# tarepan/ForwardTacotron

Measured on AMD Instinct MI355X. Metric: mel-frames/sec at batch=64 LJSpeech shapes (ForwardTacotron.generate, B*T_mel per s), higher is better.
Workload: dtype fp32; 1 GPU; c3: ForwardTacotron generate, batch=64 per GPU, phoneme lengths U{50..200}; global_batch=64, T_phonemes=200, T_mel=1368, parallelism=dp1

## Files before the change

### forwardtacotron_amd/csrc/rnn.hip

```cpp
#include "common.h"

#ifdef FTMI_RNN_STAMPS
__device__ unsigned long long ftmi_rnn_stamps[2048 * 8];
#define STAMP(i)                                                                      \
  do {                                                                                \
    if (threadIdx.x == 0) {                                                           \
      __builtin_amdgcn_sched_barrier(0);                                              \
      unsigned long long now__;                                                       \
      asm volatile("s_waitcnt vmcnt(0) lgkmcnt(0)\n\ts_memtime %0\n\ts_waitcnt lgkmcnt(0)" \
                   : "=s"(now__)::"memory");                                         \
      __builtin_amdgcn_sched_barrier(0);                                              \
      st_acc[i] += now__ - st_last;                                                   \
      st_last = now__;                                                                \
    }                                                                                 \
  } while (0)
#else
#define STAMP(i) \
  do {           \
  } while (0)
#endif
#ifdef FTMI_DIAG
#define RNN_DIAG(p) ((p).diag)
#else
#define RNN_DIAG(p) ((void)(p), 0u)
#endif

namespace {

typedef __bf16 bf16x8 __attribute__((ext_vector_type(8)));
typedef _Float16 f16x8 __attribute__((ext_vector_type(8)));

constexpr float H3_SCALE = 2048.f;
constexpr float H3_UNSCALE = 1.f / 2048.f;

constexpr int NB = 16;
constexpr int RED_STRIDE = NB + 1;
constexpr unsigned SPIN_LIMIT_DEFAULT = 1u << 22;
unsigned g_spin_limit = SPIN_LIMIT_DEFAULT;
constexpr unsigned STATUS_TIMEOUT = 4u;
constexpr int CNT_PAD = 32;
constexpr int WS_ERR = 0;
constexpr int WS_CENSUS = 1 * CNT_PAD;
constexpr int WS_ARRIVE = 9 * CNT_PAD;
constexpr int WS_FLAGS = 10 * CNT_PAD;
constexpr int FLAGS_PER_GROUP = 64;
constexpr int WS_GROUPS_OF(int ngroups) { return WS_FLAGS + ngroups * FLAGS_PER_GROUP; }

struct RnnParams {
  const float *xp;
  int64_t xp_stride;
  int T_src;
  const int32_t *index;
  const float *xp_zero;
  const float *w_hh;
  const float *b_hh;
  float *y;
  int64_t y_stride;
  const int32_t *lengths;
  float pad_value;
  float *hx;
  int B, T;
  int ngroups_total;
  int chunk0;
  int ngroups;
  int xcd_local;
  unsigned *ws;
  unsigned *status;
  unsigned spin_limit;
  int psleep;
  int diag;
};

constexpr int WS_CHUNK = 8;
static int64_t ws_chunks(int64_t B) { return (B + WS_CHUNK - 1) / WS_CHUNK; }
static int64_t ctl_bytes(int64_t nchunks) {
  return (WS_GROUPS_OF((int)(2 * nchunks)) + 2 * nchunks * CNT_PAD) * (int64_t)sizeof(unsigned);
}

static bool hx_fits(const RnnParams &p, int H, int64_t slab_words) {
  return 2 * (int64_t)p.ngroups_total * slab_words <= 2 * (2 * ws_chunks(p.B)) * NB * (int64_t)H;
}

__device__ __forceinline__ float fast_sigmoid(float x) {
  return __builtin_amdgcn_rcpf(1.0f + __expf(-x));
}
__device__ __forceinline__ float fast_tanh(float x) { return 2.0f * fast_sigmoid(2.0f * x) - 1.0f; }

__device__ __forceinline__ void split3x8(const float (&v)[8], bf16x8 &h1, bf16x8 &h2, bf16x8 &h3) {
  typedef float f32x8 __attribute__((ext_vector_type(8)));
  f32x8 x;
#pragma unroll
  for (int i = 0; i < 8; ++i) x[i] = v[i];
  h1 = __builtin_convertvector(x, bf16x8);
  const f32x8 r1 = x - __builtin_convertvector(h1, f32x8);
  h2 = __builtin_convertvector(r1, bf16x8);
  const f32x8 r2 = r1 - __builtin_convertvector(h2, f32x8);
  h3 = __builtin_convertvector(r2, bf16x8);
}

__device__ __forceinline__ void split2h8(const float (&v)[8], f16x8 &h, f16x8 &t) {
  typedef float f32x8 __attribute__((ext_vector_type(8)));
  f32x8 x;
#pragma unroll
  for (int i = 0; i < 8; ++i) x[i] = v[i];
  h = __builtin_convertvector(x, f16x8);
  t = __builtin_convertvector((x - __builtin_convertvector(h, f32x8)) * H3_SCALE, f16x8);
}

__device__ __forceinline__ unsigned h_tag(int t) { return (((unsigned)t >> 1) & 1u) ^ 1u; }

__device__ __forceinline__ unsigned xcc_id() {
  unsigned x;
  asm volatile("s_getreg_b32 %0, hwreg(HW_REG_XCC_ID)" : "=s"(x));
  return x & 7u;
}

__device__ __forceinline__ bool poll_ge(unsigned *w, unsigned target, unsigned limit) {
  unsigned spins = 0;
  while (__hip_atomic_load(w, __ATOMIC_RELAXED, __HIP_MEMORY_SCOPE_AGENT) < target) {
    __builtin_amdgcn_s_sleep(1);
    if (++spins > limit) return false;
  }
  return true;
}

__device__ __forceinline__ void report_timeout(const RnnParams &p) {
  __hip_atomic_store(p.ws + WS_ERR, 1u, __ATOMIC_RELAXED, __HIP_MEMORY_SCOPE_AGENT);
  if (p.status) atomicOr(p.status, STATUS_TIMEOUT);
}

template <int CELL, int H, int U, int WK, int MODE, bool CST = false, int NBL = NB>
__global__ __launch_bounds__(H / U == 1 ? 256 : 320, 1) void rnn_bidir_kernel(
    const RnnParams p) {
  constexpr bool X6 = MODE != 0;
  constexpr bool H3 = MODE == 2;
  constexpr int G = CELL ? 4 : 3;
  constexpr int R = G * U;
  constexpr int RB = (R + 15) / 16;
  constexpr int WR = 4 / WK;
  constexpr int RBW = RB / WR;
  constexpr int KW = H / WK;
  constexpr int NL = KW / 16;
  constexpr int KS = KW / 32;
  constexpr int KB = KW / 4;
  constexpr int BPG = H / U;
  constexpr bool LOCAL = BPG == 1;
  constexpr int CELLS = U * NB;
  constexpr bool HALFCELL = CELLS < 256;
  constexpr int CPT = HALFCELL ? 1 : CELLS / 256;
  static_assert((R % 16 == 0 || U == 8) && (U % 16 == 0 || U == 8) && H % U == 0 &&
                    RB % WR == 0 && (CELLS % 256 == 0 || CELLS == 128), "shape");
  static_assert(X6 ? (KW % 32 == 0) : (KB % 4 == 0), "K split");
  static_assert(!CST || (H3 && !LOCAL && CPT == 1 && (U == 16 || U == 8)), "compute-wave h stores");
  static_assert(U != 8 || (CST && CELL == 0 && NBL == NB), "U = 8: the spread GRU's CST form");
  static_assert(NBL == NB || (NBL == 8 && !LOCAL), "live sequences per group");
  constexpr int RR = RB * 16;
  constexpr float GSC = H3 ? H3_UNSCALE : 1.f;

  __shared__ __attribute__((aligned(16))) float red[WK * RR * RED_STRIDE];
  __shared__ __attribute__((aligned(16))) float hloc[LOCAL ? 2 * 16 * H : 4];
  __shared__ __attribute__((aligned(16))) float hstage[LOCAL ? 4 : CELLS];
  __shared__ __attribute__((aligned(16))) float ystage[LOCAL ? 4 : CELLS];
  __shared__ int s_abort, s_group, s_bi, s_mode;

  const int tid = threadIdx.x, lane = tid & 63, wave = tid >> 6;
  const int wk = wave % WK, wr = wave / WK;
  const int ls = lane >> 4, lc = lane & 15;

  if (tid == 0) {
    int mode = 0, group = blockIdx.x % p.ngroups, bi = blockIdx.x / p.ngroups, abort = 0;
    if (!LOCAL && p.xcd_local) {
      const unsigned x = xcc_id();
      const unsigned slot = __hip_atomic_fetch_add(p.ws + WS_CENSUS + x * CNT_PAD, 1u,
                                                   __ATOMIC_RELAXED, __HIP_MEMORY_SCOPE_AGENT);
      __hip_atomic_fetch_add(p.ws + WS_ARRIVE, 1u, __ATOMIC_RELAXED, __HIP_MEMORY_SCOPE_AGENT);
      if (!poll_ge(p.ws + WS_ARRIVE, gridDim.x, p.spin_limit)) {
        abort = 1;
        report_timeout(p);
      } else if (p.ngroups % 8 == 0 || (int)gridDim.x == 8 * BPG) {
        const int gpx = p.ngroups % 8 == 0 ? p.ngroups / 8 : 1;
        const unsigned per = (unsigned)gpx * BPG;
        bool balanced = true;
        for (int i = 0; i < 8; ++i)
          balanced &= __hip_atomic_load(p.ws + WS_CENSUS + i * CNT_PAD, __ATOMIC_RELAXED,
                                        __HIP_MEMORY_SCOPE_AGENT) == per;
        if (balanced) {
          mode = 1;
          group = (int)(x * gpx + slot / BPG);
          bi = (int)(slot % BPG);
        }
      }
    }
    s_mode = mode;
    s_group = group;
    s_bi = bi;
    s_abort = abort;
  }
  __syncthreads();
  if (s_abort) return;
  if (s_group >= p.ngroups || s_bi >= BPG) return;
  const int group = s_group, bi = s_bi;
  const bool xcd_mode = s_mode == 1;
  const int dir = group & 1;
  const int chunk = p.chunk0 + (group >> 1);
  const int gglob = p.chunk0 * 2 + group;
  const int u0 = bi * U;
  unsigned *cnt = p.ws + WS_GROUPS_OF(p.ngroups_total) + gglob * CNT_PAD;
  unsigned *flags = p.ws + WS_FLAGS + gglob * FLAGS_PER_GROUP;
  static_assert(BPG <= FLAGS_PER_GROUP, "flags");

  if constexpr (!LOCAL) {
    if (wave == 4) {
      constexpr int F4 = CELLS / 4;
      constexpr int FPL = F4 < 64 ? 1 : F4 / 64;
      static_assert(F4 % 64 == 0 || F4 == 32, "comm wave tiling");
      const auto rs = __builtin_amdgcn_make_buffer_rsrc(p.hx, (short)0, 0x7FFFFFF0, 0x00020000);
      const int hxp = p.ngroups_total * 16 * H * 4;
      unsigned hofs[FPL];
      int yb[FPL], k0s[FPL];
      bool ok[FPL];
#pragma unroll
      for (int i = 0; i < FPL; ++i) {
        const int f = lane + 64 * i;
        {
          const int bl = f / (U / 4);
          yb[i] = chunk * NBL + bl;
          k0s[i] = u0 + (f % (U / 4)) * 4;
          ok[i] = f < F4 && bl < NBL && yb[i] < p.B;
        }
        if constexpr (H3) {
          const int bl = f / (U / 4), rem = f % (U / 4), plane = rem & 1;
          const int k0 = u0 + (rem >> 1) * 8;
          const int kwv = k0 / KW, r = k0 % KW, q = r % 32;
          const int ln = (q >> 3) * 16 + bl;
          hofs[i] = (unsigned)((gglob * 16 * H * 2 +
                                ((kwv * NL + (r / 32) * 2 + plane) * 64 + ln) * 8) * 2);
        } else {
          const int bl = f / (U / 4);
          const int k0 = u0 + (f % (U / 4)) * 4;
          const int kwv = k0 / KW, r = k0 % KW;
          int ln, idx4;
          if constexpr (X6) {
            const int q = r % 32;
            ln = (q >> 3) * 16 + bl;
            idx4 = (r / 32) * 2 + ((q & 7) >> 2);
          } else {
            ln = (r / KB) * 16 + bl;
            idx4 = (r % KB) >> 2;
          }
          hofs[i] = (unsigned)((gglob * 16 * H + ((kwv * NL + idx4) * 64 + ln) * 4) * 4);
        }
      }
      __syncthreads();
      for (int t = 0; t < p.T; ++t) {
        const int tt = dir ? (p.T - 1 - t) : t;
        __syncthreads();
        if (s_abort) break;
        __syncthreads();
        const int soff = (t & 1) * hxp;
        typedef unsigned u32x4 __attribute__((ext_vector_type(4)));
#pragma unroll
        for (int i = 0; i < (CST ? 0 : FPL); ++i) {
          const u32x4 v = *(const u32x4 *)&hstage[(lane + 64 * i) * 4];
          if (NBL != NB && (lane + 64 * i) / (U / 4) >= NBL) continue;
          if (xcd_mode)
            __builtin_amdgcn_raw_buffer_store_b128(v, rs, hofs[i], soff, 0);
          else
            __builtin_amdgcn_raw_buffer_store_b128(v, rs, hofs[i], soff, 16);
        }
#pragma unroll
        for (int i = 0; i < FPL; ++i) {
          const f32x4 v = *(const f32x4 *)&ystage[((lane + 64 * i) % F4) * 4];
          if (ok[i]) *(f32x4 *)(p.y + ((size_t)yb[i] * p.T + tt) * p.y_stride + dir * H + k0s[i]) = v;
        }
      }
      return;
    }
  }

  const float *wdir = p.w_hh + (size_t)dir * (G * H) * H;
  bf16x8 wa[(X6 && !H3) ? RBW : 1][(X6 && !H3) ? KS : 1][3];
  f16x8 wh[H3 ? RBW : 1][H3 ? KS : 1][2];
  float wf[X6 ? 1 : RBW][X6 ? 1 : KB];
  bool wbad = false;
#pragma unroll
  for (int i = 0; i < RBW; ++i) {
    const int lrow0 = (wr * RBW + i) * 16 + lc;
    const bool rlive = lrow0 < R;
    const int lrow = rlive ? lrow0 : 0;
    const int grow = (lrow / U) * H + u0 + (lrow % U);
    const float *src = wdir + (size_t)grow * H + wk * KW;
    if constexpr (X6) {
#pragma unroll
      for (int ks = 0; ks < KS; ++ks) {
        float v[8];
        const f32x4 a = *(const f32x4 *)(src + ks * 32 + 8 * ls);
        const f32x4 b = *(const f32x4 *)(src + ks * 32 + 8 * ls + 4);
        v[0] = a.x; v[1] = a.y; v[2] = a.z; v[3] = a.w;
        v[4] = b.x; v[5] = b.y; v[6] = b.z; v[7] = b.w;
        if (!rlive)
#pragma unroll
          for (int e = 0; e < 8; ++e) v[e] = 0.f;
        if constexpr (H3) {
          split2h8(v, wh[i][ks][0], wh[i][ks][1]);
#pragma unroll
          for (int e = 0; e < 8; ++e) wbad |= !(__builtin_fabsf(v[e]) <= 65504.f);
        } else {
          split3x8(v, wa[i][ks][0], wa[i][ks][1], wa[i][ks][2]);
        }
      }
    } else {
#pragma unroll
      for (int kb = 0; kb < KB; kb += 4) {
        const f32x4 v = *(const f32x4 *)(src + ls * KB + kb);
        wf[i][kb] = v.x;
        wf[i][kb + 1] = v.y;
        wf[i][kb + 2] = v.z;
        wf[i][kb + 3] = v.w;
      }
    }
  }

  if (wbad && p.status) atomicOr(p.status, 2u);

  int cu[CPT], cb[CPT], cbl[CPT], len[CPT], hxo[CPT];
  bool cvalid[CPT];
  float hstate[CPT], cstate[CPT], bhh[CPT][G];
#pragma unroll
  for (int j = 0; j < CPT; ++j) {
    const int c = tid + 256 * j;
    cu[j] = c % U;
    const int bl = c / U;
    cbl[j] = bl;
    cb[j] = chunk * NBL + bl;
    cvalid[j] = bl < NBL && cb[j] < p.B;
    hstate[j] = 0.f;
    cstate[j] = 0.f;
    len[j] = (p.lengths && cvalid[j]) ? p.lengths[cb[j]] : p.T;
#pragma unroll
    for (int g = 0; g < G; ++g) {
      bhh[j][g] = (CELL == 0) ? p.b_hh[dir * G * H + g * H + u0 + cu[j]] : 0.f;
    }
    const int k = u0 + cu[j];
    const int kwv = k / KW, r = k % KW;
    int ln, idx4, e;
    if constexpr (X6) {
      const int q = r % 32;
      ln = (q >> 3) * 16 + bl;
      idx4 = (r / 32) * 2 + ((q & 7) >> 2);
      e = q & 3;
    } else {
      ln = (r / KB) * 16 + bl;
      idx4 = (r % KB) >> 2;
      e = r & 3;
    }
    hxo[j] = ((kwv * NL + idx4) * 64 + ln) * 4 + e;
  }

  const int slab = 16 * H;
  const auto rsrc = __builtin_amdgcn_make_buffer_rsrc(p.hx, (short)0, 0x7FFFFFF0, 0x00020000);
  const unsigned hoff = (unsigned)((gglob * slab + wk * NL * 256 + lane * 4) * 4);
  const int hx_par = p.ngroups_total * slab * 4;
  unsigned cst_off = 0;
  if constexpr (CST) {
    const int f = 16 * wave + (lane & 15);
    const int bl = f / (U / 4), rem = f % (U / 4), plane = rem & 1;
    const int k0 = u0 + (rem >> 1) * 8;
    const int kwv = k0 / KW, r = k0 % KW, q = r % 32;
    const int ln = (q >> 3) * 16 + bl;
    cst_off = (unsigned)((gglob * 16 * H * 2 + ((kwv * NL + (r / 32) * 2 + plane) * 64 + ln) * 8) * 2);
  }

  const int32_t *iptr[CPT];
  size_t brow[CPT];
#pragma unroll
  for (int j = 0; j < CPT; ++j) {
    const int b = cvalid[j] ? cb[j] : 0;
    iptr[j] = p.index ? p.index + (size_t)b * p.T : (const int32_t *)p.ws;
    brow[j] = (size_t)b * p.T_src;
  }
  const float *xcol = p.xp + dir * G * H + u0;
  const float *zcol = (p.index ? p.xp_zero : p.xp) + dir * G * H + u0;
  auto frame = [&](int t) { return dir ? (p.T - 1 - t) : t; };
  auto load_idx = [&](int t, int (&ir)[CPT]) {
    const int tt = frame(t < p.T ? t : p.T - 1);
#pragma unroll
    for (int j = 0; j < CPT; ++j) ir[j] = iptr[j][p.index ? tt : 0];
  };
  auto load_gx = [&](int t, const int (&ir)[CPT], float (&g)[CPT][G]) {
    const int tt = frame(t < p.T ? t : p.T - 1);
#pragma unroll
    for (int j = 0; j < CPT; ++j) {
      const int src = p.index ? ir[j] : tt;
      const float *row = src >= 0 ? xcol + (brow[j] + src) * p.xp_stride : zcol;
      if (RNN_DIAG(p) & 1) row = zcol;
#pragma unroll
      for (int gi = 0; gi < G; ++gi) g[j][gi] = row[gi * H + cu[j]];
    }
  };
  float g0[CPT][G], g1[CPT][G], g2[CPT][G];
  int i0[CPT], i1[CPT], i2[CPT];
  load_idx(0, i0);
  load_idx(1, i1);
  load_gx(0, i0, g0);
  load_gx(1, i1, g1);
  load_idx(2, i2);
  if (LOCAL)
    for (int i = tid; i < 16 * H; i += 256) hloc[i] = 0.f;
  __syncthreads();

#ifdef FTMI_RNN_STAMPS
  unsigned long long st_acc[6] = {0, 0, 0, 0, 0, 0}, st_last = 0;
  if (tid == 0) st_last = __builtin_amdgcn_s_memtime();
#endif

  auto step = [&](int t, const float (&gx)[CPT][G], float (&gnext)[CPT][G],
                  const int (&inext)[CPT], int (&iload)[CPT]) -> bool {
    const int tt = frame(t);
    STAMP(0);
    typedef unsigned u32x4 __attribute__((ext_vector_type(4)));
    constexpr bool HSPLIT = H3 && !LOCAL;
    float hv[HSPLIT ? 1 : NL * 4];
    u32x4 hr[NL];
    if (t == 0) {
#pragma unroll
      for (int i = 0; i < (HSPLIT ? 1 : NL * 4); ++i) hv[i] = 0.f;
#pragma unroll
      for (int i = 0; i < NL; ++i) hr[i] = (u32x4){0u, 0u, 0u, 0u};
    } else if constexpr (LOCAL) {
      const float *hb = hloc + ((t - 1) & 1) * slab + wk * NL * 256 + lane * 4;
#pragma unroll
      for (int i = 0; i < NL; ++i) {
        const f32x4 v = *(const f32x4 *)(hb + i * 256);
        hv[4 * i] = v.x;
        hv[4 * i + 1] = v.y;
        hv[4 * i + 2] = v.z;
        hv[4 * i + 3] = v.w;
      }
    } else {
      if constexpr (NBL != NB) {
#pragma unroll
        for (int i = 0; i < NL; ++i) hr[i] = (u32x4){0u, 0u, 0u, 0u};
      }
      const int soff = ((t - 1) & 1) * hx_par;
      for (int i = 0; i < p.psleep; ++i) __builtin_amdgcn_s_sleep(1);
      const unsigned tmask = HSPLIT ? 0x00010001u : 1u;
      const bool want1 = h_tag(t - 1) != 0u;
      const bool hlive = (lane & 15) < NBL;
      for (unsigned spins = 0;; ++spins) {
        asm volatile("" ::: "memory");
#pragma unroll
        for (int i = 0; i < NL; ++i)
          if ((NBL == NB || hlive) && !((RNN_DIAG(p) & 64) && i >= NL / 4))
            hr[i] = __builtin_amdgcn_raw_buffer_load_b128(rsrc, hoff + i * 1024, soff, 16);
        bool fresh;
        if (want1) {
          u32x4 a = hr[0];
#pragma unroll
          for (int i = 1; i < NL; ++i) a &= hr[i];
          fresh = ((a.x & a.y & a.z & a.w) & tmask) == tmask;
        } else {
          u32x4 o = hr[0];
#pragma unroll
          for (int i = 1; i < NL; ++i) o |= hr[i];
          fresh = ((o.x | o.y | o.z | o.w) & tmask) == 0u;
        }
        if (__all(fresh || !hlive) || (RNN_DIAG(p) & 2) != 0) break;
        if (spins > p.spin_limit) {
          if (lane == 0) {
            s_abort = 1;
            report_timeout(p);
          }
          break;
        }
        if (RNN_DIAG(p) & 16) __builtin_amdgcn_s_sleep(1);
      }
#pragma unroll
      for (int i = 0; i < (HSPLIT ? 0 : NL); ++i) {
        const f32x4 v = __builtin_bit_cast(f32x4, hr[i]);
        hv[4 * i] = v.x;
        hv[4 * i + 1] = v.y;
        hv[4 * i + 2] = v.z;
        hv[4 * i + 3] = v.w;
      }
    }
    STAMP(1);
    load_gx(t + 2, inext, gnext);
    load_idx(t + 3, iload);
    STAMP(2);

    f32x4 acc[RBW];
#pragma unroll
    for (int i = 0; i < RBW; ++i) acc[i] = (f32x4){0.f, 0.f, 0.f, 0.f};
    if constexpr (H3) {
#pragma unroll
      for (int ks = 0; ks < KS; ++ks) {
        float v[8];
#pragma unroll
        for (int e = 0; e < 8; ++e) v[e] = HSPLIT ? 0.f : hv[HSPLIT ? 0 : ks * 8 + e];
        f16x8 hh, ht;
        if constexpr (HSPLIT) {
          hh = __builtin_bit_cast(f16x8, hr[2 * ks]);
          ht = __builtin_bit_cast(f16x8, hr[2 * ks + 1]);
        } else {
          split2h8(v, hh, ht);
        }
        const f16x8 hs = hh * (_Float16)H3_SCALE;
#pragma unroll
        for (int i = 0; i < RBW; ++i) {
          f32x4 c = acc[i];
          if (!(RNN_DIAG(p) & 32)) {
            c = __builtin_amdgcn_mfma_f32_16x16x32_f16(wh[i][ks][1], hh, c, 0, 0, 0);
            c = __builtin_amdgcn_mfma_f32_16x16x32_f16(wh[i][ks][0], ht, c, 0, 0, 0);
          }
          c = __builtin_amdgcn_mfma_f32_16x16x32_f16(wh[i][ks][0], hs, c, 0, 0, 0);
          acc[i] = c;
        }
      }
    } else if constexpr (X6) {
#pragma unroll
      for (int ks = 0; ks < KS; ++ks) {
        float v[8];
#pragma unroll
        for (int e = 0; e < 8; ++e) v[e] = hv[ks * 8 + e];
        bf16x8 h1, h2, h3;
        split3x8(v, h1, h2, h3);
#pragma unroll
        for (int i = 0; i < RBW; ++i) {
          f32x4 c = acc[i];
          c = __builtin_amdgcn_mfma_f32_16x16x32_bf16(wa[i][ks][2], h1, c, 0, 0, 0);
          c = __builtin_amdgcn_mfma_f32_16x16x32_bf16(wa[i][ks][1], h2, c, 0, 0, 0);
          c = __builtin_amdgcn_mfma_f32_16x16x32_bf16(wa[i][ks][0], h3, c, 0, 0, 0);
          c = __builtin_amdgcn_mfma_f32_16x16x32_bf16(wa[i][ks][1], h1, c, 0, 0, 0);
          c = __builtin_amdgcn_mfma_f32_16x16x32_bf16(wa[i][ks][0], h2, c, 0, 0, 0);
          c = __builtin_amdgcn_mfma_f32_16x16x32_bf16(wa[i][ks][0], h1, c, 0, 0, 0);
          acc[i] = c;
        }
      }
    } else {
#pragma unroll
      for (int kb = 0; kb < KB; ++kb)
#pragma unroll
        for (int i = 0; i < RBW; ++i)
          acc[i] = __builtin_amdgcn_mfma_f32_16x16x4f32(wf[i][kb], hv[kb], acc[i], 0, 0, 0);
    }
#pragma unroll
    for (int i = 0; i < RBW; ++i)
#pragma unroll
      for (int e = 0; e < 4; ++e)
        red[(wk * RR + (wr * RBW + i) * 16 + ls * 4 + e) * RED_STRIDE + lc] = acc[i][e];
    __syncthreads();
    if (!LOCAL && s_abort) return false;
    STAMP(3);

#pragma unroll
    for (int j = 0; j < CPT; ++j) {
      if (HALFCELL && tid >= CELLS) continue;
      const int bl = cbl[j];
      float gs[G], gi[G];
#pragma unroll
      for (int g = 0; g < G; ++g) {
        const int row = g * U + cu[j];
        float sum = red[row * RED_STRIDE + bl];
#pragma unroll
        for (int w = 1; w < WK; ++w) sum += red[(w * RR + row) * RED_STRIDE + bl];
        gs[g] = sum;
        gi[g] = gx[j][g];
      }
      float hn;
      if (RNN_DIAG(p) & 128) {
        hn = 0.25f * (fmaf(gs[0], GSC, gi[0]) + fmaf(gs[1], GSC, gi[1]) +
                      fmaf(gs[2], GSC, gi[2]) + (CELL ? fmaf(gs[G - 1], GSC, gi[G - 1]) : 0.f));
        hn = fminf(fmaxf(hn, -0.9f), 0.9f);
      } else if (CELL == 0) {
        const float r = fast_sigmoid(gi[0] + fmaf(gs[0], GSC, bhh[j][0]));
        const float z = fast_sigmoid(gi[1] + fmaf(gs[1], GSC, bhh[j][1]));
        const float n = fast_tanh(gi[2] + r * fmaf(gs[2], GSC, bhh[j][2]));
        hn = n + z * (hstate[j] - n);
      } else {
        const float ig = fast_sigmoid(fmaf(gs[0], GSC, gi[0]));
        const float fg = fast_sigmoid(fmaf(gs[1], GSC, gi[1]));
        const float gg = fast_tanh(fmaf(gs[2], GSC, gi[2]));
        const float og = fast_sigmoid(fmaf(gs[3], GSC, gi[3]));
        cstate[j] = fg * cstate[j] + ig * gg;
        hn = og * fast_tanh(cstate[j]);
      }
      if (tt >= len[j]) {
        hn = 0.f;
        cstate[j] = 0.f;
      }
      if constexpr (HSPLIT) {
        const unsigned short tg = (unsigned short)h_tag(t);
        const _Float16 h16 = __builtin_bit_cast(
            _Float16, (unsigned short)((__builtin_bit_cast(unsigned short, (_Float16)hn) & 0xFFFEu) | tg));
        const _Float16 t16 = __builtin_bit_cast(
            _Float16, (unsigned short)((__builtin_bit_cast(unsigned short,
                                                           (_Float16)((hn - (float)h16) * H3_SCALE)) &
                                        0xFFFEu) | tg));
        _Float16 *hs16 = (_Float16 *)hstage;
        const int base = ((bl * (U / 8) + cu[j] / 8) * 2) * 8 + (cu[j] % 8);
        hs16[base] = h16;
        hs16[base + 8] = t16;
      } else if constexpr (!LOCAL) {
        hn = __uint_as_float((__float_as_uint(hn) & ~1u) | h_tag(t));
      }
      const float yout = tt >= len[j] ? p.pad_value : hn;
      hstate[j] = hn;
      if constexpr (LOCAL) {
        if (cvalid[j]) {
          hloc[(t & 1) * slab + hxo[j]] = hn;
          p.y[((size_t)cb[j] * p.T + tt) * p.y_stride + dir * H + u0 + cu[j]] = yout;
        }
      } else {
        const int c = bl * U + cu[j];
        if constexpr (!HSPLIT) hstage[c] = hn;
        ystage[c] = yout;
      }
    }
    if constexpr (CST) {
      __builtin_amdgcn_fence(__ATOMIC_RELEASE, "wavefront");
      __builtin_amdgcn_wave_barrier();
      if (lane < 16 && (16 * wave + lane) / (U / 4) < NBL) {
        typedef unsigned u32x4 __attribute__((ext_vector_type(4)));
        const u32x4 v = *(const u32x4 *)&hstage[(16 * wave + lane) * 4];
        if (xcd_mode)
          __builtin_amdgcn_raw_buffer_store_b128(v, rsrc, cst_off, (t & 1) * hx_par, 0);
        else
          __builtin_amdgcn_raw_buffer_store_b128(v, rsrc, cst_off, (t & 1) * hx_par, 16);
      }
    }
    STAMP(4);
    __syncthreads();
    STAMP(5);
    return true;
  };

  for (int t = 0; t < p.T; t += 3) {
    if (!step(t, g0, g2, i2, i0)) break;
    if (t + 1 >= p.T || !step(t + 1, g1, g0, i0, i1)) break;
    if (t + 2 >= p.T || !step(t + 2, g2, g1, i1, i2)) break;
  }
#ifdef FTMI_RNN_STAMPS
  if (tid == 0)
    for (int i = 0; i < 6; ++i) ftmi_rnn_stamps[blockIdx.x * 8 + i] = st_acc[i];
#endif
}

constexpr int GV_KSEG = 8;
constexpr int GV_RPT = 2;

template <int CELL, int H, int U, int NBV, int KSEG = GV_KSEG>
__global__ __launch_bounds__((CELL ? 4 : 3) * U / GV_RPT * KSEG) void rnn_gemv_kernel(
    const RnnParams p) {
  constexpr int G = CELL ? 4 : 3;
  constexpr int R = G * U;
  constexpr int NT = R / GV_RPT * KSEG;
  constexpr int SEG = H / KSEG;
  constexpr int SEGP = SEG + 4;
  constexpr int BPG = H / U;
  constexpr int HF4 = H / 4;
  static_assert(R % GV_RPT == 0 && SEG % 4 == 0 && U * NBV <= NT && NT % 64 == 0, "shape");
  static_assert(BPG <= FLAGS_PER_GROUP, "group size");
  __shared__ __attribute__((aligned(16))) float hl[2][NBV * KSEG * SEGP];
  __shared__ float red[R][NBV];
  __shared__ int s_abort, s_group, s_bi, s_mode;

  const int tid = threadIdx.x, lane = tid & 63;
  const int ks = tid % KSEG, rg = tid / KSEG;

  if (tid == 0) {
    int mode = 0, group = blockIdx.x % p.ngroups, bi = blockIdx.x / p.ngroups, abort = 0;
    if (p.xcd_local) {
      const unsigned x = xcc_id();
      const unsigned slot = __hip_atomic_fetch_add(p.ws + WS_CENSUS + x * CNT_PAD, 1u,
                                                   __ATOMIC_RELAXED, __HIP_MEMORY_SCOPE_AGENT);
      __hip_atomic_fetch_add(p.ws + WS_ARRIVE, 1u, __ATOMIC_RELAXED, __HIP_MEMORY_SCOPE_AGENT);
      if (!poll_ge(p.ws + WS_ARRIVE, gridDim.x, p.spin_limit)) {
        abort = 1;
        report_timeout(p);
      } else if ((int)gridDim.x == 8 * BPG) {
        bool balanced = true;
        for (int i = 0; i < 8; ++i)
          balanced &= __hip_atomic_load(p.ws + WS_CENSUS + i * CNT_PAD, __ATOMIC_RELAXED,
                                        __HIP_MEMORY_SCOPE_AGENT) == (unsigned)BPG;
        if (balanced) {
          mode = 1;
          group = (int)x;
          bi = (int)slot;
        }
      }
    }
    s_mode = mode;
    s_group = group;
    s_bi = bi;
    s_abort = abort;
  }
  __syncthreads();
  if (s_abort) return;
  if (s_group >= p.ngroups || s_bi >= BPG) return;
  const int dir = s_group, u0 = s_bi * U;
  const bool xcd_mode = s_mode == 1;

  const float *wdir = p.w_hh + (size_t)dir * (G * H) * H;
  float w[GV_RPT][SEG];
#pragma unroll
  for (int i = 0; i < GV_RPT; ++i) {
    const int r = rg * GV_RPT + i;
    const float *src = wdir + (size_t)((r / U) * H + u0 + r % U) * H + ks * SEG;
#pragma unroll
    for (int j = 0; j < SEG; j += 4) {
      const f32x4 v = *(const f32x4 *)(src + j);
      w[i][j] = v.x;
      w[i][j + 1] = v.y;
      w[i][j + 2] = v.z;
      w[i][j + 3] = v.w;
    }
  }

  const bool is_cell = tid < U * p.B;
  const int cu = tid % U, cb = is_cell ? tid / U : 0;
  float hstate = 0.f, cstate = 0.f, bhh[G];
#pragma unroll
  for (int g = 0; g < G; ++g) bhh[g] = (CELL == 0) ? p.b_hh[dir * G * H + g * H + u0 + cu] : 0.f;
  const int len = (p.lengths && is_cell) ? p.lengths[cb] : p.T;
  const int32_t *iptr = p.index ? p.index + (size_t)cb * p.T : (const int32_t *)p.ws;
  const float *xcol = p.xp + dir * G * H + u0 + cu;
  const float *zcol = (p.index ? p.xp_zero : p.xp) + dir * G * H + u0 + cu;
  auto frame = [&](int t) { return dir ? (p.T - 1 - t) : t; };
  auto load_idx = [&](int t) -> int { return iptr[p.index ? frame(t < p.T ? t : p.T - 1) : 0]; };
  auto load_gx = [&](int t, int ir, float (&g)[G]) {
    const int tt = frame(t < p.T ? t : p.T - 1);
    const int src = p.index ? ir : tt;
    const float *row = src >= 0 ? xcol + ((size_t)cb * p.T_src + src) * p.xp_stride : zcol;
#pragma unroll
    for (int gi = 0; gi < G; ++gi) g[gi] = row[gi * H];
  };
  float g0[G], g1[G], g2[G];
  int i0 = load_idx(0), i1 = load_idx(1);
  load_gx(0, i0, g0);
  load_gx(1, i1, g1);
  int i2 = load_idx(2);

  const auto rsrc = __builtin_amdgcn_make_buffer_rsrc(p.hx, (short)0, 0x7FFFFFF0, 0x00020000);
  const int par_bytes = 2 * NBV * H * 4;
  const int nf4 = p.B * HF4;
  const unsigned hx_off = (unsigned)(((dir * NBV + cb) * H + u0 + cu) * 4);

  auto step = [&](int t, const float (&gx)[G], float (&gnext)[G], int inext, int &iload) -> bool {
    const int tt = frame(t);
    float *hb = hl[t & 1];
    const unsigned want = h_tag(t - 1);
    for (int f = tid; f < nf4; f += NT) {
      const int b = f / HF4, k = (f - b * HF4) * 4;
      f32x4 v = {0.f, 0.f, 0.f, 0.f};
      if (t > 0) {
        const unsigned off = (unsigned)(((dir * NBV + b) * H + k) * 4);
        const int soff = ((t - 1) & 1) * par_bytes;
        for (unsigned spins = 0;; ++spins) {
          asm volatile("" ::: "memory");
          typedef unsigned u32x4 __attribute__((ext_vector_type(4)));
          const u32x4 r = __builtin_amdgcn_raw_buffer_load_b128(rsrc, off, soff, 16);
          const bool fresh = want ? ((r.x & r.y & r.z & r.w) & 1u) != 0u
                                  : ((r.x | r.y | r.z | r.w) & 1u) == 0u;
          if (fresh || (RNN_DIAG(p) & 2)) {
            v = __builtin_bit_cast(f32x4, r);
            break;
          }
          if (spins > p.spin_limit) {
            s_abort = 1;
            report_timeout(p);
            break;
          }
        }
      }
      *(f32x4 *)&hb[b * KSEG * SEGP + (k / SEG) * SEGP + k % SEG] = v;
    }
    for (int f = nf4 + tid; f < NBV * HF4; f += NT) {
      const int b = f / HF4, k = (f - b * HF4) * 4;
      *(f32x4 *)&hb[b * KSEG * SEGP + (k / SEG) * SEGP + k % SEG] = (f32x4){0.f, 0.f, 0.f, 0.f};
    }
    __syncthreads();
    if (s_abort) return false;
    if (is_cell) {
      load_gx(t + 2, inext, gnext);
      iload = load_idx(t + 3);
    }
    float acc[GV_RPT][NBV];
#pragma unroll
    for (int i = 0; i < GV_RPT; ++i)
#pragma unroll
      for (int b = 0; b < NBV; ++b) acc[i][b] = 0.f;
#pragma unroll
    for (int b = 0; b < NBV; ++b) {
      const float *hs = hb + b * KSEG * SEGP + ks * SEGP;
#pragma unroll
      for (int j = 0; j < SEG; j += 4) {
        const f32x4 hv = *(const f32x4 *)(hs + j);
#pragma unroll
        for (int i = 0; i < GV_RPT; ++i) {
          acc[i][b] = fmaf(w[i][j], hv.x, acc[i][b]);
          acc[i][b] = fmaf(w[i][j + 1], hv.y, acc[i][b]);
          acc[i][b] = fmaf(w[i][j + 2], hv.z, acc[i][b]);
          acc[i][b] = fmaf(w[i][j + 3], hv.w, acc[i][b]);
        }
      }
    }
#pragma unroll
    for (int i = 0; i < GV_RPT; ++i)
#pragma unroll
      for (int b = 0; b < NBV; ++b) {
        float v = acc[i][b];
        v += __shfl_xor(v, 1);
        v += __shfl_xor(v, 2);
        v += __shfl_xor(v, 4);
        if constexpr (KSEG == 16) v += __shfl_xor(v, 8);
        acc[i][b] = v;
      }
    if (ks < GV_RPT)
#pragma unroll
      for (int b = 0; b < NBV; ++b)
        red[rg * GV_RPT + ks][b] = ks == 0 ? acc[0][b] : acc[GV_RPT - 1][b];
    __syncthreads();
    if (is_cell) {
      float gs[G];
#pragma unroll
      for (int g = 0; g < G; ++g) gs[g] = red[g * U + cu][cb];
      float hn;
      if (CELL == 0) {
        const float r = fast_sigmoid(gx[0] + (gs[0] + bhh[0]));
        const float z = fast_sigmoid(gx[1] + (gs[1] + bhh[1]));
        const float n = fast_tanh(gx[2] + r * (gs[2] + bhh[2]));
        hn = n + z * (hstate - n);
      } else {
        const float ig = fast_sigmoid(gx[0] + gs[0]);
        const float fg = fast_sigmoid(gx[1] + gs[1]);
        const float gg = fast_tanh(gx[2] + gs[2]);
        const float og = fast_sigmoid(gx[3] + gs[3]);
        cstate = fg * cstate + ig * gg;
        hn = og * fast_tanh(cstate);
      }
      if (tt >= len) {
        hn = 0.f;
        cstate = 0.f;
      }
      hn = __uint_as_float((__float_as_uint(hn) & ~1u) | h_tag(t));
      hstate = hn;
      const float yout = tt >= len ? p.pad_value : hn;
      const int soff = (t & 1) * par_bytes;
      if (xcd_mode)
        __builtin_amdgcn_raw_buffer_store_b32(__float_as_uint(hn), rsrc, hx_off, soff, 0);
      else
        __builtin_amdgcn_raw_buffer_store_b32(__float_as_uint(hn), rsrc, hx_off, soff, 16);
      p.y[((size_t)cb * p.T + tt) * p.y_stride + dir * H + u0 + cu] = yout;
    }
    return true;
  };

  for (int t = 0; t < p.T; t += 3) {
    if (!step(t, g0, g2, i2, i0)) break;
    if (t + 1 >= p.T || !step(t + 1, g1, g0, i0, i1)) break;
    if (t + 2 >= p.T || !step(t + 2, g2, g1, i1, i2)) break;
  }
}

template <int CELL, int H, int U, int KSEG = GV_KSEG>
int launch_gemv(RnnParams p, int max_blocks, hipStream_t s) {
  constexpr int BPG = H / U;
  constexpr int NT = (CELL ? 4 : 3) * U / GV_RPT * KSEG;
  if (8 * BPG > max_blocks) return FTMI_E_UNSUPPORTED;
  p.chunk0 = 0;
  p.ngroups = 2;
  const int nblk = p.xcd_local ? 8 * BPG : 2 * BPG;
#define FTMI_GEMV_LAUNCH(NBV_)                                                             \
  if (int rc = ftmi_resident_ok((const void *)rnn_gemv_kernel<CELL, H, U, NBV_, KSEG>, nblk, NT, 0)) \
    return rc;                                                                               \
  hipLaunchKernelGGL((rnn_gemv_kernel<CELL, H, U, NBV_, KSEG>), dim3(nblk), dim3(NT), 0, s, p); \
  break;
  switch (p.B) {
    case 1: FTMI_GEMV_LAUNCH(1)
    case 2: FTMI_GEMV_LAUNCH(2)
    default: FTMI_GEMV_LAUNCH(4)
  }
#undef FTMI_GEMV_LAUNCH
  FTMI_CHECK_LAUNCH();
  return FTMI_OK;
}

template <int CELL, int H, int U, int WK, int MODE, bool CST = false, int NBL = NB>
int launch_rnn(RnnParams p, int nchunks, int max_blocks, hipStream_t s) {
  if (NBL != NB) {
    nchunks = (p.B + NBL - 1) / NBL;
    p.ngroups_total = 2 * nchunks;
  }
  if (!hx_fits(p, H, (int64_t)NB * H)) return FTMI_E_SHAPE;
  constexpr int BPG = H / U;
  int max_groups = (max_blocks / BPG) & ~1;
  if (max_groups < 2) return FTMI_E_UNSUPPORTED;
  for (int c0 = 0; c0 < nchunks; c0 += max_groups / 2) {
    const int nc = (nchunks - c0) < max_groups / 2 ? (nchunks - c0) : max_groups / 2;
    p.chunk0 = c0;
    p.ngroups = 2 * nc;
    if (c0 > 0) {
      hipError_t e = hipMemsetAsync(p.ws + WS_CENSUS, 0, (WS_FLAGS - WS_CENSUS) * 4, s);
      if (e != hipSuccess) return (int)e;
    }
    static const int pad_env = [] {
      const char *v = getenv("FTMI_RNN_PAD");
      return v ? atoi(v) : 1;
    }();
    int nblk = p.ngroups * BPG;
    if (BPG > 1 && pad_env && p.xcd_local && p.ngroups < 8 && 8 * BPG <= max_blocks)
      nblk = 8 * BPG;
    if (int rc = ftmi_resident_ok((const void *)rnn_bidir_kernel<CELL, H, U, WK, MODE, CST, NBL>,
                                  nblk, BPG == 1 ? 256 : 320, 0))
      return rc;
    hipLaunchKernelGGL((rnn_bidir_kernel<CELL, H, U, WK, MODE, CST, NBL>), dim3(nblk),
                       dim3(BPG == 1 ? 256 : 320), 0, s, p);
    FTMI_CHECK_LAUNCH();
  }
  return FTMI_OK;
}

int device_cu_count() {
  static int cus = 0;
  if (cus == 0) {
    int dev = 0;
    if (hipGetDevice(&dev) != hipSuccess ||
        hipDeviceGetAttribute(&cus, hipDeviceAttributeMultiprocessorCount, dev) != hipSuccess ||
        cus <= 0)
      cus = 256;
  }
  return cus;
}

}

constexpr int GV_MAXB = 4;
static bool gemv_path(int cell, int B, int H) {
  const char *v = getenv("FTMI_RNN_GEMV");
  const int env = v ? atoi(v) : 1;
  return env && B <= GV_MAXB && ((cell == 1 && H == 512) || (cell == 0 && (H == 64 || H == 128 || H == 256)));
}
static int xcd_local_env() {
  static const int v = [] {
    const char *e = getenv("FTMI_RNN_XCD_LOCAL");
    return e ? atoi(e) : 1;
  }();
  return v;
}

static int rnn_units(int cell, int H, int mma) {
  if (cell == 0 && H == 64) {
    static const int u64 = [] {
      const char *v = getenv("FTMI_RNN_U64");
      return v ? atoi(v) : 32;
    }();
    return (mma == 2 && u64 == 32) ? 32 : 64;
  }
  return 16;
}

static bool cst_enabled() {
  const char *v = getenv("FTMI_RNN_CSTORE");
  return !(v && atoi(v) == 0);
}
static int legacy_nbl(int cell, int B, int H, int mma, bool spread, int maxb) {
  const char *v = getenv("FTMI_RNN_NB");
  if (!spread || mma != 2 || cell != 0 || H != 256 || !cst_enabled() ||
      (v && atoi(v) == 16))
    return NB;
  return 2 * ((B + 7) / 8) * (H / 16) <= maxb ? 8 : NB;
}

static bool u8_path(int cell, int B, int H, int mma, bool spread, int maxb) {
  if (!spread || mma != 2 || !cst_enabled() || cell != 0 || H != 256) return false;
  const char *v = getenv("FTMI_RNN_U8");
  if (v && atoi(v) == 0) return false;
  const int ngroups = 2 * ((B + NB - 1) / NB);
  return (ngroups < 8 ? 8 : ngroups) * (H / 8) <= maxb;
}

extern "C" int32_t ftmi_rnn_blocks(int32_t cell, int32_t B, int32_t H, int32_t mma) {
  if (B <= 0 || H <= 0 || H % 16 != 0) return 0;
  const bool spread = (mma & FTMI_RNN_SPREAD) != 0;
  mma &= 0xFF;
  if (gemv_path(cell, B, H)) return (xcd_local_env() ? 8 : 2) * (H / 16);
  if (u8_path(cell, B, H, mma, spread, device_cu_count())) {
    const int ngroups = 2 * ((B + NB - 1) / NB);
    return (ngroups < 8 && xcd_local_env() ? 8 : ngroups) * (H / 8);
  }
  const int bpg = H / rnn_units(cell, H, mma);
  const int maxb = device_cu_count();
  const int max_groups = (maxb / bpg) & ~1;
  if (max_groups < 2) return 0;
  const int nbl = legacy_nbl(cell, B, H, mma, spread, maxb);
  const int nchunks = (B + nbl - 1) / nbl;
  const int ngroups = 2 * (nchunks < max_groups / 2 ? nchunks : max_groups / 2);
  int nblk = ngroups * bpg;
  if (bpg > 1 && ngroups < 8 && 8 * bpg <= maxb) nblk = 8 * bpg;
  return nblk;
}

extern "C" int64_t ftmi_rnn_workspace_bytes(int32_t B, int32_t H, int32_t cell) {
  (void)cell;
  if (B <= 0 || H <= 0) return 0;
  const int64_t nchunks = ws_chunks(B);
  return ctl_bytes(nchunks) + 2 * (2 * nchunks) * NB * (int64_t)H * (int64_t)sizeof(float);
}


extern "C" uint32_t ftmi_set_rnn_spin_limit(uint32_t limit) {
  const unsigned prev = g_spin_limit;
  g_spin_limit = limit ? limit : SPIN_LIMIT_DEFAULT;
  return prev;
}

extern "C" int64_t ftmi_rnn_error_offset(int32_t B) {
  (void)B;
  return WS_ERR * (int64_t)sizeof(unsigned);
}

static int rnn_setup(RnnParams &p, int B, int T, int H, int cell, const float *w_hh,
                     const float *b_hh, const int32_t *lengths, float pad_value, float *y,
                     int64_t y_stride, uint32_t *status, void *sync, hipStream_t s,
                     int &nchunks) {
  nchunks = (B + NB - 1) / NB;
  const int64_t ctl = ctl_bytes(ws_chunks(B));
  const int64_t wsb = ftmi_rnn_workspace_bytes(B, H, cell);
  hipError_t e = hipMemsetAsync(sync, 0, (size_t)wsb, s);
  if (e != hipSuccess) return (int)e;
  p.w_hh = w_hh;
  p.b_hh = b_hh;
  p.y = y;
  p.y_stride = y_stride;
  p.lengths = lengths;
  p.pad_value = pad_value;
  p.B = B;
  p.T = T;
  p.ngroups_total = 2 * nchunks;
  p.xcd_local = xcd_local_env();
  p.ws = (unsigned *)sync;
  p.hx = (float *)((char *)sync + ctl);
  p.status = status;
  p.spin_limit = g_spin_limit;
#ifdef FTMI_DIAG
  static const int diag_env = [] {
    const char *v = getenv("FTMI_RNN_DIAG");
    return v ? atoi(v) : 0;
  }();
  p.diag = diag_env;
#endif
  static const int psleep_env = [] {
    const char *v = getenv("FTMI_RNN_PSLEEP");
    return v ? atoi(v) : -1;
  }();
  p.psleep = psleep_env < 0 ? 3 : psleep_env;
  return FTMI_OK;
}

static int u8_psleep() {
  const char *v = getenv("FTMI_RNN_PSLEEP");
  return v ? atoi(v) : 6;
}

extern "C" int ftmi_rnn_bidir(int32_t cell, int32_t B, int32_t T, int32_t H, const float *xp,
                              int64_t xp_stride, int32_t T_src, const int32_t *index,
                              const float *xp_zero, const float *w_hh, const float *b_hh,
                              const int32_t *lengths, float pad_value, float *y,
                              int64_t y_stride, int32_t mma, uint32_t *status, void *sync,
                              ftmi_stream_t stream) {
  if (!xp || !w_hh || !y || !sync) return FTMI_E_ARG;
  if (B <= 0 || T <= 0 || H <= 0 || T_src <= 0) return FTMI_E_ARG;
  const bool spread = (mma & FTMI_RNN_SPREAD) != 0;
  mma &= ~FTMI_RNN_SPREAD;
  if (mma < 0 || mma > 2) return FTMI_E_ARG;
  if (cell == 0 && !b_hh) return FTMI_E_ARG;
  if (index && !xp_zero) return FTMI_E_ARG;
  if (!index && T_src != T) return FTMI_E_SHAPE;
  if (!ftmi_aligned16(w_hh) || !ftmi_aligned16(sync)) return FTMI_E_ALIGN;
  if (!ftmi_aligned16(y) || (y_stride & 3)) return FTMI_E_ALIGN;
  if (cell == 1 ? H != 512 : (cell != 0 || (H != 64 && H != 128 && H != 256)))
    return FTMI_E_UNSUPPORTED;
  hipStream_t s = ftmi_hs(stream);
  RnnParams p = {};
  int nchunks = 0;
  const int rc = rnn_setup(p, B, T, H, cell, w_hh, b_hh, lengths, pad_value, y, y_stride,
                           status, sync, s, nchunks);
  if (rc != FTMI_OK) return rc;
  p.xp = xp;
  p.xp_stride = xp_stride;
  p.T_src = T_src;
  p.index = index;
  p.xp_zero = xp_zero;
  const int maxb = device_cu_count();
  if (gemv_path(cell, B, H)) {
    const char *kv = getenv("FTMI_RNN_GEMV_KSEG");
    const bool k8 = kv && atoi(kv) == 8;
    if (cell == 1) return k8 ? launch_gemv<1, 512, 16>(p, maxb, s) : launch_gemv<1, 512, 16, 16>(p, maxb, s);
    if (H == 256) return k8 ? launch_gemv<0, 256, 16>(p, maxb, s) : launch_gemv<0, 256, 16, 16>(p, maxb, s);
    if (H == 128) return launch_gemv<0, 128, 16>(p, maxb, s);
    return launch_gemv<0, 64, 16>(p, maxb, s);
  }
#define FTMI_RNN_MODES(CELL_, H_, U_, WKX_, WKF_)                                   \
  switch (mma) {                                                                    \
    case 2: return launch_rnn<CELL_, H_, U_, WKX_, 2>(p, nchunks, maxb, s);          \
    case 1: return launch_rnn<CELL_, H_, U_, WKX_, 1>(p, nchunks, maxb, s);          \
    default: return launch_rnn<CELL_, H_, U_, WKF_, 0>(p, nchunks, maxb, s);         \
  }
  if (cell == 0 && H == 64) {
    if (rnn_units(cell, H, mma) == 32) return launch_rnn<0, 64, 32, 2, 2>(p, nchunks, maxb, s);
    FTMI_RNN_MODES(0, 64, 64, 2, 4)
  }
  if (cell == 0 && H == 128) FTMI_RNN_MODES(0, 128, 16, 4, 4)
  if (mma == 2 && cst_enabled() && ((cell == 1 && H == 512) || (cell == 0 && H == 256))) {
    const bool nb8 = legacy_nbl(cell, B, H, mma, spread, maxb) == 8;
    if (u8_path(cell, B, H, mma, spread, maxb)) {
      p.psleep = u8_psleep();
      return launch_rnn<0, 256, 8, 4, 2, true>(p, nchunks, maxb, s);
    }
    if (cell == 1) return launch_rnn<1, 512, 16, 4, 2, true>(p, nchunks, maxb, s);
    return nb8 ? launch_rnn<0, 256, 16, 4, 2, true, 8>(p, nchunks, maxb, s)
               : launch_rnn<0, 256, 16, 4, 2, true>(p, nchunks, maxb, s);
  }
  if (cell == 0 && H == 256) FTMI_RNN_MODES(0, 256, 16, 4, 4)
  if (cell == 1 && H == 512) FTMI_RNN_MODES(1, 512, 16, 4, 4)
#undef FTMI_RNN_MODES
  return FTMI_E_UNSUPPORTED;
}

#ifdef FTMI_RNN_STAMPS
extern "C" int ftmi_debug_rnn_stamps(unsigned long long *host, int n) {
  return (int)hipMemcpyFromSymbol(host, HIP_SYMBOL(ftmi_rnn_stamps),
                                  sizeof(unsigned long long) * (size_t)n, 0, hipMemcpyDeviceToHost);
}
#endif
```

Before: 11.27 million mel-frames/s.

## Add single-workgroup GRU kernel for H=64 with in-block sync and writer wave

Adds a GRU recurrence kernel for hidden size 64 in which each batch chunk and direction runs in one workgroup. Hidden state is exchanged through double-buffered LDS with __syncthreads, replacing cross-block global flag synchronization. The recurrent matmul uses split-fp16 MFMA, and a dedicated extra wave streams outputs from LDS staging to global memory. The workspace memset shrinks to just the error counter. The path covers only unpadded, non-indexed calls, and runs far fewer blocks, so each direction gets less parallelism.

```diff
diff --git a/forwardtacotron_amd/csrc/rnn.hip b/forwardtacotron_amd/csrc/rnn.hip
--- a/forwardtacotron_amd/csrc/rnn.hip
+++ b/forwardtacotron_amd/csrc/rnn.hip
@@ -646,6 +646,160 @@
 #endif
 }
 
+template <int H, bool VEC>
+__global__ __launch_bounds__((H / 16 + 1) * 64, 1) void gru_wg_kernel(const RnnParams p) {
+  constexpr int G = 3;
+  constexpr int NW = H / 16;
+  constexpr int KS = H / 32;
+  constexpr int YS = H + 4;
+  static_assert(H == 64, "shape");
+  __shared__ __attribute__((aligned(16))) _Float16 himg[2 * KS * 2 * 64 * 8];
+  __shared__ __attribute__((aligned(16))) float ystage[2 * NB * YS];
+
+  const int tid = threadIdx.x, lane = tid & 63, wave = tid >> 6;
+  const int ls = lane >> 4, lc = lane & 15;
+  const int dir = blockIdx.x & 1, chunk = blockIdx.x >> 1;
+
+  if (wave == NW) {
+    constexpr int FPL = NB * H / 4 / 64;
+    float *yp[FPL];
+    int so[FPL];
+    bool ok[FPL];
+#pragma unroll
+    for (int i = 0; i < FPL; ++i) {
+      const int f = lane + 64 * i, bl = f / (H / 4), k0 = (f % (H / 4)) * 4;
+      const int b = chunk * NB + bl;
+      ok[i] = b < p.B;
+      yp[i] = p.y + (size_t)(ok[i] ? b : 0) * p.T * p.y_stride + dir * H + k0;
+      so[i] = bl * YS + k0;
+    }
+    __syncthreads();
+    for (int t = 0; t < p.T; ++t) {
+      const int tt = dir ? (p.T - 1 - t) : t;
+      __syncthreads();
+      const float *ys = ystage + (t & 1) * NB * YS;
+#pragma unroll
+      for (int i = 0; i < FPL; ++i) {
+        const f32x4 v = *(const f32x4 *)(ys + so[i]);
+        if (ok[i]) *(f32x4 *)(yp[i] + (size_t)tt * p.y_stride) = v;
+      }
+    }
+    return;
+  }
+
+  const float *wdir = p.w_hh + (size_t)dir * (G * H) * H;
+  f16x8 wh[G][KS][2];
+  bool wbad = false;
+#pragma unroll
+  for (int g = 0; g < G; ++g) {
+    const float *src = wdir + (size_t)(g * H + 16 * wave + lc) * H + 8 * ls;
+#pragma unroll
+    for (int ks = 0; ks < KS; ++ks) {
+      float v[8];
+      const f32x4 a = *(const f32x4 *)(src + ks * 32);
+      const f32x4 b = *(const f32x4 *)(src + ks * 32 + 4);
+      v[0] = a.x; v[1] = a.y; v[2] = a.z; v[3] = a.w;
+      v[4] = b.x; v[5] = b.y; v[6] = b.z; v[7] = b.w;
+      split2h8(v, wh[g][ks][0], wh[g][ks][1]);
+#pragma unroll
+      for (int e = 0; e < 8; ++e) wbad |= !(__builtin_fabsf(v[e]) <= 65504.f);
+    }
+  }
+  if (wbad && p.status) atomicOr(p.status, 2u);
+
+  const int u0 = 16 * wave + 4 * ls;
+  const int b = chunk * NB + lc;
+  const int bc = b < p.B ? b : 0;
+  float bhh[G][4], hstate[4];
+#pragma unroll
+  for (int g = 0; g < G; ++g)
+#pragma unroll
+    for (int e = 0; e < 4; ++e) bhh[g][e] = p.b_hh[dir * G * H + g * H + u0 + e];
+#pragma unroll
+  for (int e = 0; e < 4; ++e) hstate[e] = 0.f;
+
+  const auto xrs = __builtin_amdgcn_make_buffer_rsrc(const_cast<float *>(p.xp), (short)0,
+                                                     0x7FFFFFF0, 0x00020000);
+  const unsigned xoff = (unsigned)(((size_t)bc * p.T * p.xp_stride + dir * G * H + u0) * 4);
+  auto frame = [&](int t) { return dir ? (p.T - 1 - t) : t; };
+  auto load_gx = [&](int t, f32x4 (&g)[G]) {
+    const int row = (int)(frame(t < p.T ? t : p.T - 1) * p.xp_stride * 4);
+#pragma unroll
+    for (int gi = 0; gi < G; ++gi) {
+      if constexpr (VEC) {
+        g[gi] = __builtin_bit_cast(
+            f32x4, __builtin_amdgcn_raw_buffer_load_b128(xrs, xoff + gi * H * 4, row, 0));
+      } else {
+#pragma unroll
+        for (int e = 0; e < 4; ++e)
+          g[gi][e] = __builtin_bit_cast(
+              float, __builtin_amdgcn_raw_buffer_load_b32(xrs, xoff + (gi * H + e) * 4, row, 0));
+      }
+    }
+  };
+  f32x4 g0[G], g1[G], g2[G];
+  load_gx(0, g0);
+  load_gx(1, g1);
+
+  _Float16 *hw = himg + (((wave >> 1) * 2) * 64 + (2 * (wave & 1) + (ls >> 1)) * 16 + lc) * 8 +
+                 4 * (ls & 1);
+  const _Float16 *hr = himg + lane * 8;
+  float *yw = ystage + lc * YS + u0;
+  constexpr int HPAR = KS * 2 * 64 * 8;
+  for (int i = tid; i < HPAR; i += NW * 64) ((unsigned *)himg)[i] = 0u;
+  __syncthreads();
+
+  auto step = [&](int t, const f32x4 (&gx)[G], f32x4 (&gnext)[G]) {
+    load_gx(t + 2, gnext);
+    f32x4 acc[G];
+#pragma unroll
+    for (int g = 0; g < G; ++g) acc[g] = (f32x4){0.f, 0.f, 0.f, 0.f};
+    const _Float16 *hp = hr + ((t + 1) & 1) * HPAR;
+#pragma unroll
+    for (int ks = 0; ks < KS; ++ks) {
+      const f16x8 hh = *(const f16x8 *)(hp + (ks * 2) * 64 * 8);
+      const f16x8 ht = *(const f16x8 *)(hp + (ks * 2 + 1) * 64 * 8);
+      const f16x8 hs = hh * (_Float16)H3_SCALE;
+#pragma unroll
+      for (int g = 0; g < G; ++g)
+        acc[g] = __builtin_amdgcn_mfma_f32_16x16x32_f16(wh[g][ks][1], hh, acc[g], 0, 0, 0);
+#pragma unroll
+      for (int g = 0; g < G; ++g)
+        acc[g] = __builtin_amdgcn_mfma_f32_16x16x32_f16(wh[g][ks][0], ht, acc[g], 0, 0, 0);
+#pragma unroll
+      for (int g = 0; g < G; ++g)
+        acc[g] = __builtin_amdgcn_mfma_f32_16x16x32_f16(wh[g][ks][0], hs, acc[g], 0, 0, 0);
+    }
+    typedef _Float16 f16x4 __attribute__((ext_vector_type(4)));
+    f32x4 hn4;
+    f16x4 h4, t4;
+#pragma unroll
+    for (int e = 0; e < 4; ++e) {
+      const float r = fast_sigmoid(gx[0][e] + fmaf(acc[0][e], H3_UNSCALE, bhh[0][e]));
+      const float z = fast_sigmoid(gx[1][e] + fmaf(acc[1][e], H3_UNSCALE, bhh[1][e]));
+      const float n = fast_tanh(gx[2][e] + r * fmaf(acc[2][e], H3_UNSCALE, bhh[2][e]));
+      const float hn = n + z * (hstate[e] - n);
+      hstate[e] = hn;
+      hn4[e] = hn;
+      h4[e] = (_Float16)hn;
+      t4[e] = (_Float16)((hn - (float)h4[e]) * H3_SCALE);
+    }
+    _Float16 *hq = hw + (t & 1) * HPAR;
+    *(f16x4 *)hq = h4;
+    *(f16x4 *)(hq + 64 * 8) = t4;
+    *(f32x4 *)(yw + (t & 1) * NB * YS) = hn4;
+    __syncthreads();
+  };
+
+  for (int t = 0; t < p.T; t += 3) {
+    step(t, g0, g2);
+    if (t + 1 >= p.T) break;
+    step(t + 1, g1, g0);
+    if (t + 2 >= p.T) break;
+    step(t + 2, g2, g1);
+  }
+}
+
 constexpr int GV_KSEG = 8;
 constexpr int GV_RPT = 2;
 
@@ -921,6 +1075,18 @@
   return FTMI_OK;
 }
 
+template <int H>
+int launch_gru_wg(RnnParams p, int nchunks, hipStream_t s) {
+  const bool vec = ftmi_aligned16(p.xp) && (p.xp_stride & 3) == 0;
+  const dim3 grid(2 * nchunks), block((H / 16 + 1) * 64);
+  if (vec)
+    hipLaunchKernelGGL((gru_wg_kernel<H, true>), grid, block, 0, s, p);
+  else
+    hipLaunchKernelGGL((gru_wg_kernel<H, false>), grid, block, 0, s, p);
+  FTMI_CHECK_LAUNCH();
+  return FTMI_OK;
+}
+
 int device_cu_count() {
   static int cus = 0;
   if (cus == 0) {
@@ -941,6 +1107,11 @@
   const int env = v ? atoi(v) : 1;
   return env && B <= GV_MAXB && ((cell == 1 && H == 512) || (cell == 0 && (H == 64 || H == 128 || H == 256)));
 }
+static bool wg_path(int cell, int B, int H, int mma) {
+  if (cell != 0 || H != 64 || mma != 2 || gemv_path(cell, B, H)) return false;
+  const char *v = getenv("FTMI_RNN_WG");
+  return !(v && atoi(v) == 0);
+}
 static int xcd_local_env() {
   static const int v = [] {
     const char *e = getenv("FTMI_RNN_XCD_LOCAL");
@@ -985,6 +1156,7 @@
   const bool spread = (mma & FTMI_RNN_SPREAD) != 0;
   mma &= 0xFF;
   if (gemv_path(cell, B, H)) return (xcd_local_env() ? 8 : 2) * (H / 16);
+  if (wg_path(cell, B, H, mma)) return 2 * ((B + NB - 1) / NB);
   if (u8_path(cell, B, H, mma, spread, device_cu_count())) {
     const int ngroups = 2 * ((B + NB - 1) / NB);
     return (ngroups < 8 && xcd_local_env() ? 8 : ngroups) * (H / 8);
@@ -1023,10 +1195,11 @@
 static int rnn_setup(RnnParams &p, int B, int T, int H, int cell, const float *w_hh,
                      const float *b_hh, const int32_t *lengths, float pad_value, float *y,
                      int64_t y_stride, uint32_t *status, void *sync, hipStream_t s,
-                     int &nchunks) {
+                     int &nchunks, bool err_only) {
   nchunks = (B + NB - 1) / NB;
   const int64_t ctl = ctl_bytes(ws_chunks(B));
-  const int64_t wsb = ftmi_rnn_workspace_bytes(B, H, cell);
+  const int64_t wsb = err_only ? CNT_PAD * (int64_t)sizeof(unsigned)
+                               : ftmi_rnn_workspace_bytes(B, H, cell);
   hipError_t e = hipMemsetAsync(sync, 0, (size_t)wsb, s);
   if (e != hipSuccess) return (int)e;
   p.w_hh = w_hh;
@@ -1084,8 +1257,10 @@
   hipStream_t s = ftmi_hs(stream);
   RnnParams p = {};
   int nchunks = 0;
+  const bool wg = !index && !lengths && wg_path(cell, B, H, mma) &&
+                  (int64_t)B * T * xp_stride * 4 < 0x7FFFFFF0ll;
   const int rc = rnn_setup(p, B, T, H, cell, w_hh, b_hh, lengths, pad_value, y, y_stride,
-                           status, sync, s, nchunks);
+                           status, sync, s, nchunks, wg);
   if (rc != FTMI_OK) return rc;
   p.xp = xp;
   p.xp_stride = xp_stride;
@@ -1093,6 +1268,7 @@
   p.index = index;
   p.xp_zero = xp_zero;
   const int maxb = device_cu_count();
+  if (wg) return launch_gru_wg<64>(p, nchunks, s);
   if (gemv_path(cell, B, H)) {
     const char *kv = getenv("FTMI_RNN_GEMV_KSEG");
     const bool k8 = kv && atoi(kv) == 8;
```

Result: slower. 11.05 million mel-frames/s (-2.0%).
